# marella/ctransformers

Hardware: NVIDIA H100
Metric: decode tokens/s Llama-2-7B Q4_K_M b=1 (higher is better)
Workload: dtype int8 (q4_K/q6_K weights x q8_K activations, mma.sync u8 x s8 -> exact int32), fp32 combine in the reference's order

## Files before the change

### ctransformers_b200/csrc/attention.cuh

```cuda
#pragma once
#include <cmath>
#include <vector>

#include "device_types.cuh"

namespace ctb {

__device__ __forceinline__ void k4_scale_min(int j, const uint8_t* q, int& sc, int& m) {
  if (j < 4) { sc = q[j] & 63; m = q[j + 4] & 63; }
  else { sc = (q[j + 4] & 0xF) | ((q[j - 4] >> 6) << 4); m = (q[j + 4] >> 4) | ((q[j] >> 6) << 4); }
}

template <bool Q3 = true>
__device__ __forceinline__ float dequant_elem(int type, const uint8_t* row, int e) {
  if (Q3 && type == GT_Q3_K) {
    const uint8_t* blk = row + (size_t)(e >> 8) * 110;
    const int r = e & 255, n = r >> 7, j = (r & 127) >> 5, l = r & 31, is = 8 * n + 2 * j + (l >> 4);
    const int w = is >> 2, b = is & 3;
    const int lo = w & 1 ? blk[100 + b] : blk[96 + b];
    const int sc = ((w < 2 ? lo : lo >> 4) & 0xF) | (((blk[104 + b] >> (2 * w)) & 3) << 4);
    const int q = ((blk[32 + 32 * n + l] >> (2 * j)) & 3) - ((blk[l] >> (4 * n + j)) & 1 ? 0 : 4);
    return __fmul_rn(__fmul_rn(h2f((uint16_t)(blk[108] | (blk[109] << 8))), (float)(sc - 32)), (float)q);
  }
  switch (type) {
    case GT_F32: return ((const float*)row)[e];
    case GT_F16: return h2f(((const uint16_t*)row)[e]);
    case GT_Q4_0: {
      const uint8_t* blk = row + (size_t)(e >> 5) * 18;
      const int r = e & 31;
      const float d = h2f((uint16_t)(blk[0] | (blk[1] << 8)));
      const int byte = blk[2 + (r & 15)];
      const int nib = r < 16 ? (byte & 0xF) : (byte >> 4);
      return __fmul_rn((float)(nib - 8), d);
    }
    case GT_Q5_0: {
      const uint8_t* blk = row + (size_t)(e >> 5) * 22;
      const int r = e & 31;
      const float d = h2f((uint16_t)(blk[0] | (blk[1] << 8)));
      const uint32_t qh = (uint32_t)blk[2] | ((uint32_t)blk[3] << 8) | ((uint32_t)blk[4] << 16) | ((uint32_t)blk[5] << 24);
      const int byte = blk[6 + (r & 15)];
      const int nib = r < 16 ? (byte & 0xF) : (byte >> 4);
      return __fmul_rn((float)((nib | (int)(((qh >> r) & 1u) << 4)) - 16), d);
    }
    case GT_Q4_1: case GT_Q5_1: {
      const bool q5 = type == GT_Q5_1;
      const uint8_t* blk = row + (size_t)(e >> 5) * (q5 ? 24 : 20);
      const int r = e & 31;
      const float d = h2f((uint16_t)(blk[0] | (blk[1] << 8)));
      const float m = h2f((uint16_t)(blk[2] | (blk[3] << 8)));
      const int byte = blk[(q5 ? 8 : 4) + (r & 15)];
      int q = r < 16 ? (byte & 0xF) : (byte >> 4);
      if (q5) q |= ((blk[4 + (r >> 3)] >> (r & 7)) & 1) << 4;
      return __fmaf_rn((float)q, d, m);
    }
    case GT_Q8_0: {
      const uint8_t* blk = row + (size_t)(e >> 5) * 34;
      const float d = h2f((uint16_t)(blk[0] | (blk[1] << 8)));
      return __fmul_rn((float)(int8_t)blk[2 + (e & 31)], d);
    }
    case GT_Q4_K: case GT_Q5_K: {
      const bool q5 = type == GT_Q5_K;
      const uint8_t* blk = row + (size_t)(e >> 8) * (q5 ? 176 : 144);
      const int r = e & 255, j = r >> 6, within = r & 63, sub = 2 * j + (within >> 5), l = within & 31;
      const float d = h2f((uint16_t)(blk[0] | (blk[1] << 8)));
      const float dmin = h2f((uint16_t)(blk[2] | (blk[3] << 8)));
      int sc, m;
      k4_scale_min(sub, blk + 4, sc, m);
      const uint8_t* qs = blk + (q5 ? 48 : 16);
      const int byte = qs[32 * j + l];
      int q = (sub & 1) ? (byte >> 4) : (byte & 0xF);
      if (q5 && (blk[16 + l] & (1 << sub))) q += 16;
      return __fsub_rn(__fmul_rn(__fmul_rn(d, (float)sc), (float)q), __fmul_rn(dmin, (float)m));
    }
    case GT_Q6_K: {
      const uint8_t* blk = row + (size_t)(e >> 8) * 210;
      const uint8_t* ql = blk; const uint8_t* qh = blk + 128; const int8_t* sc = (const int8_t*)(blk + 192);
      const float d = h2f((uint16_t)(blk[208] | (blk[209] << 8)));
      const int r = e & 255, n = r >> 7, rr = r & 127, k = rr >> 5, l = rr & 31, is = l >> 4;
      const int byte = ql[64 * n + ((k & 1) ? 32 : 0) + l];
      const int nib = (k >= 2) ? (byte >> 4) : (byte & 0xF);
      const int hb = (qh[32 * n + l] >> (2 * k)) & 3;
      const int q = (int)(int8_t)(nib | (hb << 4)) - 32;
      return __fmul_rn(__fmul_rn(d, (float)sc[8 * n + is + 2 * k]), (float)q);
    }
  }
  return 0.f;
}

struct EmbedParams { const uint8_t* table; size_t row_bytes; const int* tokens; float* out; int type, K, n_vocab; };

template <bool Q3 = true>
__device__ __forceinline__ void embed_row(const EmbedParams& em, int tok, float* out, int tid, int nt) {
  const uint8_t* row = em.table + (size_t)min(max(tok, 0), em.n_vocab - 1) * em.row_bytes;
  for (int e = tid; e < em.K; e += nt) out[e] = dequant_elem<Q3>(em.type, row, e);
}

static __global__ void k_embed(const EmbedParams em) {
  embed_row(em, em.tokens[blockIdx.x], em.out + (size_t)blockIdx.x * em.K, threadIdx.x, blockDim.x);
}

__host__ __device__ inline int kv_ctx_pad(int n_ctx) { return (n_ctx + 255) & ~255; }
__host__ __device__ inline int k_stride(int hd) { return (hd + 7) & ~7; }
template <bool GEN = true>
__host__ __device__ inline size_t k_row(int kv_head, int pos, int n_ctx, int hd) { return ((size_t)kv_head * n_ctx + pos) * (GEN ? k_stride(hd) : hd); }
__host__ __device__ inline size_t v_chan(int kv_head, int c, int n_ctx, int hd) { return ((size_t)kv_head * hd + c) * kv_ctx_pad(n_ctx); }
template <bool GEN = true>
__host__ __device__ inline int k_perm(int e, int hd) {
  if (!GEN) return (e & 31) * (hd >> 5) + (e >> 5);
  const int np = hd & ~31;
  return e < np ? (e & 31) * (np >> 5) + (e >> 5) : e;
}
__host__ __device__ inline int v_perm(int t) { return (t & ~255) + (t & 31) * 8 + ((t >> 5) & 7); }

inline std::vector<float2> rope_table(int n_pos, int hd, int n_rot, float freq_base, float freq_scale) {
  const int half = hd / 2;
  std::vector<float2> tab((size_t)n_pos * half);
  const float theta_scale = powf(freq_base, -2.0f / n_rot);
  for (int p = 0; p < n_pos; p++) {
    float theta = freq_scale * (float)p;
    for (int i = 0; i < half; i++) {
      tab[(size_t)p * half + i] = make_float2(cosf(theta), sinf(theta));
      theta *= theta_scale;
    }
  }
  return tab;
}

__device__ __forceinline__ void rope_pair(float x0, float x1, float2 cs, int neox, float& o0, float& o1) {
  if (neox) {
    o0 = __fmaf_rn(x0, cs.x, -__fmul_rn(x1, cs.y));
    o1 = __fmaf_rn(x0, cs.y, __fmul_rn(x1, cs.x));
  } else {
    o0 = __fsub_rn(__fmul_rn(x0, cs.x), __fmul_rn(x1, cs.y));
    o1 = __fadd_rn(__fmul_rn(x0, cs.y), __fmul_rn(x1, cs.x));
  }
}

__device__ __forceinline__ void rope_head_pair(const float* x, int i, int hd, int neox, float2 cs, int& i0, int& i1, float& o0, float& o1) {
  i0 = neox ? i : 2 * i;
  i1 = neox ? i + hd / 2 : 2 * i + 1;
  rope_pair(__ldcg(x + i0), __ldcg(x + i1), cs, neox, o0, o1);
}

template <bool GEN = true>
__device__ __forceinline__ void rope_k_pair(const float* x, int i, int hd, int neox, float2 cs, uint16_t* row, uint16_t* row2 = nullptr) {
  int i0, i1;
  float o0, o1;
  rope_head_pair(x, i, hd, neox, cs, i0, i1, o0, o1);
  const uint16_t h0 = f2h(o0), h1 = f2h(o1);
  row[k_perm<GEN>(i0, hd)] = h0; row[k_perm<GEN>(i1, hd)] = h1;
  if (row2) { row2[k_perm<GEN>(i0, hd)] = h0; row2[k_perm<GEN>(i1, hd)] = h1; }
}

struct AttnParams {
  const float* q;
  const float* k;
  const float* v;
  uint16_t* kc;
  uint16_t* vc;
  float* out;
  const uint16_t* exp_tab;
  const float2* rope;
  const int* state;
  float kq_scale;
  int n_head, n_kv, hd, n_ctx, q_stride, kv_stride, neox;
};

constexpr int ATTN_THREADS = 512;
constexpr int ATTN_CH = 32;
__host__ __device__ inline int attn_groups(int hd) { return (hd + ATTN_CH - 1) / ATTN_CH; }

struct AttnScratch { float* sc; uint16_t *p16, *q16, *k16, *v16; size_t bytes; };
template <bool GEN = true>
__host__ __device__ inline AttnScratch attn_scratch(uint8_t* base, int n_ctx, int hd, bool cur) {
  const size_t cp = kv_ctx_pad(n_ctx), ks = GEN ? k_stride(hd) : hd, end_q = cp * 6 + ks * 2;
  AttnScratch s;
  s.sc = (float*)base;
  s.p16 = (uint16_t*)(base + cp * 4);
  s.q16 = s.p16 + cp;
  s.k16 = cur ? s.q16 + ks : nullptr;
  s.v16 = cur ? s.k16 + ks : nullptr;
  s.bytes = cur ? end_q + ks * 2 + (size_t)hd * 2 : end_q;
  return s;
}
__host__ __device__ inline size_t attn_smem_bytes(int n_ctx, int hd) { return attn_scratch(nullptr, n_ctx, hd, true).bytes + (size_t)ATTN_CH * 4; }

__device__ __forceinline__ float attn_reduce_f32x8(float v) {
  v = v + __shfl_xor_sync(0xffffffffu, v, 16);
  v = v + __shfl_xor_sync(0xffffffffu, v, 8);
  v = v + __shfl_xor_sync(0xffffffffu, v, 4);
  v = v + __shfl_xor_sync(0xffffffffu, v, 1);
  v = v + __shfl_xor_sync(0xffffffffu, v, 2);
  return v;
}

template <int BAR, int NT>
__device__ __forceinline__ void attn_bar() {
  if constexpr (NT == 32) __syncwarp();
  else asm volatile("bar.sync %0, %1;" ::"n"(BAR), "n"(NT) : "memory");
}
template <int NT>
__device__ __forceinline__ int attn_tid() { return NT == 32 ? (int)(threadIdx.x & 31) : (int)threadIdx.x; }

struct AttnPos { int pos, T, n_vec, lim; };
__device__ __forceinline__ AttnPos attn_pos(const AttnParams& p, const int* st) {
  AttnPos a;
  a.pos = st[1];
  if (a.pos >= p.n_ctx) { a.T = 0; a.n_vec = 0; a.lim = 0; return a; }
  a.T = a.pos + 1;
  a.n_vec = max(a.T, min(st[3], p.n_ctx)) & ~31;
  a.lim = min(a.T, a.n_vec);
  return a;
}

template <int NT>
__device__ __forceinline__ float2 attn_cs0(const AttnParams& p, int pos) {
  const int i = attn_tid<NT>();
  return i < p.hd / 2 ? p.rope[(size_t)pos * (p.hd / 2) + i] : make_float2(1.f, 0.f);
}

template <int NT, bool GEN>
__device__ __forceinline__ void attn_stage(const AttnParams& p, const AttnScratch& s, int n, int h, int cg, int pos, float2 cs0) {
  const int hd = p.hd, tid = attn_tid<NT>(), group = p.n_head / p.n_kv, kvh = h / group;
  const bool kv_writer = (h % group) == 0;
  const float* qv = p.q + (size_t)n * p.q_stride + (size_t)h * hd;
  const float* kv = p.k + (size_t)n * p.kv_stride + (size_t)kvh * hd;
  const float* vv = p.v + (size_t)n * p.kv_stride + (size_t)kvh * hd;
  uint16_t* kd = (kv_writer && cg == 0) ? p.kc + k_row<GEN>(kvh, pos, p.n_ctx, hd) : nullptr;
  for (int i = tid; i < hd / 2; i += NT) {
    const float2 cs = i == tid ? cs0 : p.rope[(size_t)pos * (hd / 2) + i];
    rope_k_pair<GEN>(qv, i, hd, p.neox, cs, s.q16);
    if (s.k16) rope_k_pair<GEN>(kv, i, hd, p.neox, cs, s.k16, kd);
  }
  if (s.k16) {
    for (int c = tid; c < hd; c += NT) {
      const uint16_t hv = f2h(__ldcg(vv + c));
      s.v16[c] = hv;
      if (kv_writer && c / ATTN_CH == cg) p.vc[v_chan(kvh, c, p.n_ctx, hd) + v_perm(pos)] = hv;
    }
  }
}

template <int PER>
struct KLane { uint32_t w[(PER + 1) / 2]; };
template <int PER>
__device__ __forceinline__ KLane<PER> attn_klane(const uint16_t* row) {
  const uint16_t* p = row + (threadIdx.x & 31) * PER;
  KLane<PER> k;
  if constexpr (PER == 8) {
    const uint4 v = *(const uint4*)p;
    k.w[0] = v.x; k.w[1] = v.y; k.w[2] = v.z; k.w[3] = v.w;
  } else if constexpr (PER == 4) {
    const uint2 v = *(const uint2*)p;
    k.w[0] = v.x; k.w[1] = v.y;
  } else if constexpr (PER % 2 == 0) {
#pragma unroll
    for (int i = 0; i < PER / 2; i++) k.w[i] = ((const uint32_t*)p)[i];
  } else {
#pragma unroll
    for (int i = 0; i < PER / 2; i++) k.w[i] = (uint32_t)p[2 * i] | ((uint32_t)p[2 * i + 1] << 16);
    k.w[PER / 2] = p[PER - 1];
  }
  return k;
}
template <int PER>
__device__ __forceinline__ uint16_t klane_elem(const KLane<PER>& k, int e) { return (uint16_t)((k.w[e >> 1] >> ((e & 1) * 16)) & 0xffff); }
template <int PER>
__device__ __forceinline__ void attn_k8(KLane<PER> (&kk)[8], const uint16_t* rows, int stride, int t0, int n, int skip) {
#pragma unroll
  for (int i = 0; i < 8; i++) {
    const int t = min(t0 + i, n - 1);
    kk[i] = t == skip ? KLane<PER>{} : attn_klane<PER>(rows + (size_t)t * stride);
  }
}

template <int PER, bool TAIL>
__device__ __forceinline__ void attn_scores_per(const uint16_t* rows, int hd, int n, int t_first, int t_step, const uint16_t* q16, float kq_scale, float* sc,
                                                int cur_t, const uint16_t* cur, const KLane<PER> (*pre)[8]) {
  constexpr int NP = PER * 32;
  constexpr int R = PER > 4 ? 4 : 8;
  const int lane = threadIdx.x & 31;
  const int stride = TAIL ? k_stride(hd) : NP, tail = TAIL ? hd - NP : 0;
  const KLane<PER> qq = attn_klane<PER>(q16);
  float q[PER];
#pragma unroll
  for (int e = 0; e < PER; e++) q[e] = h2f(klane_elem(qq, e));
  const float qt = (TAIL && lane < tail) ? h2f(q16[NP + lane]) : 0.f;
  for (int t0 = t_first; t0 < n; t0 += t_step) {
#pragma unroll
    for (int r0 = 0; r0 < 8; r0 += R) {
      KLane<PER> kk[R];
      uint16_t kt[R];
      if (pre && t0 == t_first) {
#pragma unroll
        for (int i = 0; i < R; i++) kk[i] = (*pre)[r0 + i];
      } else {
#pragma unroll
        for (int i = 0; i < R; i++) {
          const int t = min(t0 + r0 + i, n - 1);
          kk[i] = t == cur_t ? KLane<PER>{} : attn_klane<PER>(rows + (size_t)t * stride);
        }
      }
      if constexpr (TAIL) {
#pragma unroll
        for (int i = 0; i < R; i++) {
          const int t = min(t0 + r0 + i, n - 1);
          kt[i] = lane < tail ? (t == cur_t ? cur : rows + (size_t)t * stride)[NP + lane] : (uint16_t)0;
        }
      }
#pragma unroll
      for (int i = 0; i < R; i++)
        if (min(t0 + r0 + i, n - 1) == cur_t) kk[i] = attn_klane<PER>(cur);
#pragma unroll
      for (int i = 0; i < R; i++) {
        float s = 0.f;
#pragma unroll
        for (int e = 0; e < PER; e++) s = __fmaf_rn(h2f(klane_elem(kk[i], e)), q[e], s);
        s = attn_reduce_f32x8(s);
        if constexpr (TAIL) {
          const float term = __fmul_rn(h2f(kt[i]), qt);
          double sumf = (double)s;
          for (int l = 0; l < tail; l++) sumf += (double)__shfl_sync(0xffffffffu, term, l);
          s = (float)sumf;
        }
        if (lane == 0 && t0 + r0 + i < n) sc[t0 + r0 + i] = __fmul_rn(s, kq_scale);
      }
    }
  }
}
#define ATTN_PER_DISPATCH(GEN, hd, F)                             \
  do {                                                            \
    if constexpr (!(GEN)) {                                       \
      if ((hd) == 128) F(4, false);                               \
      else F(2, false);                                           \
    } else {                                                      \
      switch ((hd) >> 5) {                                        \
        case 1: F(1, true); break;                                \
        case 2: F(2, true); break;                                \
        case 3: F(3, true); break;                                \
        case 4: F(4, true); break;                                \
        case 5: F(5, true); break;                                \
        case 6: F(6, true); break;                                \
        case 7: F(7, true); break;                                \
        default: F(8, true); break;                               \
      }                                                           \
    }                                                             \
  } while (0)
template <bool GEN>
__device__ __forceinline__ void attn_scores(int hd, const uint16_t* rows, int n, int t_first, int t_step, const uint16_t* q16, float kq_scale, float* sc,
                                            int cur_t = -1, const uint16_t* cur = nullptr) {
#define ATTN_SCORES_F(PER, TAIL) attn_scores_per<PER, TAIL>(rows, hd, n, t_first, t_step, q16, kq_scale, sc, cur_t, cur, nullptr)
  ATTN_PER_DISPATCH(GEN, hd, ATTN_SCORES_F);
#undef ATTN_SCORES_F
}

template <int NT, int BAR>
__device__ __forceinline__ void attn_softmax(float* sc, uint16_t* p16, int T, const uint16_t* exp_tab, float* red_f, double* red_d) {
  constexpr int NW = NT / 32;
  const int tid = attn_tid<NT>(), warp = tid >> 5, lane = tid & 31;
  float mx = -INFINITY;
  for (int t = tid; t < T; t += NT) mx = fmaxf(mx, sc[t]);
  mx = warp_max(mx);
  if constexpr (NW > 1) {
    if (lane == 0) red_f[warp] = mx;
    attn_bar<BAR, NT>();
    mx = red_f[0];
#pragma unroll
    for (int w = 1; w < NW; w++) mx = fmaxf(mx, red_f[w]);
  }
  double sum = 0.0;
  for (int t = tid; t < T; t += NT) {
    const float val = h2f(__ldg(exp_tab + f2h(__fsub_rn(sc[t], mx))));
    sc[t] = val;
    sum += (double)val;
  }
  sum = warp_sum(sum);
  if constexpr (NW > 1) {
    if (lane == 0) red_d[warp] = sum;
    attn_bar<BAR, NT>();
    sum = 0.0;
#pragma unroll
    for (int w = 0; w < NW; w++) sum += red_d[w];
  }
  const float inv = (float)(1.0 / sum);
  const int t_end = (T + 255) & ~255;
  for (int t = tid; t < t_end; t += NT) p16[v_perm(t)] = t < T ? f2h(__fmul_rn(sc[t], inv)) : (uint16_t)0;
  attn_bar<BAR, NT>();
}

__device__ __forceinline__ float attn_vp(const uint16_t* vrow, const uint16_t* p16, const AttnPos& a, int cur_t, uint16_t vcur, const uint4* pre = nullptr) {
  const int lane = threadIdx.x & 31;
  float s = 0.f;
  for (int ch = 0; ch * 256 < a.lim; ch++) {
    uint4 vv;
    if (pre && ch == 0) vv = pre[0];
    else if (pre && ch == 1) vv = pre[1];
    else vv = *(const uint4*)(vrow + ch * 256 + lane * 8);
    const uint4 pp = *(const uint4*)(p16 + ch * 256 + lane * 8);
    const uint32_t vw[4] = {vv.x, vv.y, vv.z, vv.w}, pw[4] = {pp.x, pp.y, pp.z, pp.w};
#pragma unroll
    for (int i = 0; i < 8; i++) {
      const int t = ch * 256 + 32 * i + lane;
      if (t < a.lim) {
        uint16_t vh = (uint16_t)((vw[i >> 1] >> ((i & 1) * 16)) & 0xffff);
        const uint16_t ph = (uint16_t)((pw[i >> 1] >> ((i & 1) * 16)) & 0xffff);
        if (t == cur_t) vh = vcur;
        s = __fmaf_rn(h2f(vh), h2f(ph), s);
      }
    }
  }
  s = attn_reduce_f32x8(s);
  double sumf = (double)s;
  const int n_left = a.T - a.n_vec;
  if (n_left > 0) {
    const int i = (a.n_vec >> 8) * 256 + lane * 8 + ((a.n_vec & 255) >> 5);
    const uint16_t vh = a.n_vec + lane == cur_t ? vcur : vrow[i];
    const float term = __fmul_rn(h2f(vh), h2f(p16[i]));
    for (int l = 0; l < n_left; l++) sumf += (double)__shfl_sync(0xffffffffu, term, l);
  }
  return (float)sumf;
}

template <int NT, int BAR, bool PDLWAIT, int PER, bool TAIL>
__device__ __forceinline__ void attn_body_per(const AttnParams& p, uint8_t* smem, const int h, const int n, const int cg, const AttnPos& a,
                                              float* red_f, double* red_d) {
  constexpr int NW = NT / 32;
  const int hd = p.hd, kvh = h / (p.n_head / p.n_kv), nch = TAIL ? min(ATTN_CH, hd - cg * ATTN_CH) : ATTN_CH;
  const int warp = threadIdx.x >> 5, lane = threadIdx.x & 31;
  const AttnScratch s = attn_scratch<TAIL>(smem, p.n_ctx, hd, true);
  const uint16_t* krows = p.kc + k_row<TAIL>(kvh, 0, p.n_ctx, hd);
  constexpr int CPW = (ATTN_CH + NW - 1) / NW;
  uint4 vpre[CPW][2];
  constexpr bool KPRE = PER <= 4;
  KLane<PER> kpre[8];
#pragma unroll
  for (int j = 0; j < CPW; j++)
#pragma unroll
    for (int ch = 0; ch < 2; ch++)
      vpre[j][ch] = (ch * 256 < a.lim && warp + j * NW < nch) ? *(const uint4*)(p.vc + v_chan(kvh, cg * ATTN_CH + warp + j * NW, p.n_ctx, hd) + ch * 256 + lane * 8) : make_uint4(0, 0, 0, 0);
  if constexpr (KPRE) attn_k8<PER>(kpre, krows, TAIL ? k_stride(hd) : PER * 32, warp * 8, a.T, a.pos);
  const float2 cs0 = attn_cs0<NT>(p, a.pos);
  if (PDLWAIT) pdl_wait();

  attn_stage<NT, TAIL>(p, s, n, h, cg, a.pos, cs0);
  attn_bar<BAR, NT>();
  attn_scores_per<PER, TAIL>(krows, hd, a.T, warp * 8, NW * 8, s.q16, p.kq_scale, s.sc, a.pos, s.k16, KPRE ? &kpre : nullptr);
  attn_bar<BAR, NT>();
  attn_softmax<NT, BAR>(s.sc, s.p16, a.T, p.exp_tab, red_f, red_d);
#pragma unroll
  for (int j = 0; j < CPW; j++) {
    const int cc = warp + j * NW;
    if (cc >= nch) break;
    const int c = cg * ATTN_CH + cc;
    const float o = attn_vp(p.vc + v_chan(kvh, c, p.n_ctx, hd), s.p16, a, a.pos, s.v16[c], vpre[j]);
    if (lane == 0) p.out[(size_t)n * p.n_head * hd + (size_t)h * hd + c] = o;
  }
}
template <int NT>
__device__ __forceinline__ void attn_body_red(float*& red_f, double*& red_d) {
  __shared__ float rf[NT / 32];
  __shared__ double rd[NT / 32];
  red_f = rf;
  red_d = rd;
}
template <int NT, int BAR, bool PDLWAIT, bool GEN>
__device__ __forceinline__ void attn_body(const AttnParams& p, uint8_t* smem, const int h, const int n, const int cg, const int* st) {
  float* red_f;
  double* red_d;
  attn_body_red<NT>(red_f, red_d);
  const AttnPos a = attn_pos(p, st);
  if (a.T == 0) return;
#define ATTN_BODY_F(PER, TAIL) attn_body_per<NT, BAR, PDLWAIT, PER, TAIL>(p, smem, h, n, cg, a, red_f, red_d)
  ATTN_PER_DISPATCH(GEN, p.hd, ATTN_BODY_F);
#undef ATTN_BODY_F
}

template <bool GEN>
static __global__ void __launch_bounds__(ATTN_THREADS) k_attn(const AttnParams p) {
  extern __shared__ __align__(16) uint8_t smem[];
  pdl_trigger();
  attn_body<ATTN_THREADS, 0, true, GEN>(p, smem, blockIdx.x, blockIdx.y, blockIdx.z, p.state);
}
inline void (*attn_kernel(int hd))(const AttnParams) { return attn_fast_hd(hd) ? k_attn<false> : k_attn<true>; }

template <int NT, int BAR, bool CG>
__device__ __forceinline__ void block_argmax(const float* logits, int n, float* bv , int* bi , float& best, int& idx) {
  best = -INFINITY;
  idx = 0x7fffffff;
#pragma unroll(CG ? 4 : 1)
  for (int i = threadIdx.x; i < n; i += NT) {
    const float v = CG ? __ldcg(logits + i) : logits[i];
    if (v > best) { best = v; idx = i; }
  }
#pragma unroll
  for (int o = 16; o > 0; o >>= 1) {
    const float ov = __shfl_xor_sync(0xffffffffu, best, o);
    const int oi = __shfl_xor_sync(0xffffffffu, idx, o);
    if (ov > best || (ov == best && oi < idx)) { best = ov; idx = oi; }
  }
  if ((threadIdx.x & 31) == 0) { bv[threadIdx.x >> 5] = best; bi[threadIdx.x >> 5] = idx; }
  bar_sync<BAR, NT>();
  if (threadIdx.x == 0) {
    for (int w = 1; w < NT / 32; w++)
      if (bv[w] > best || (bv[w] == best && bi[w] < idx)) { best = bv[w]; idx = bi[w]; }
    const float x0 = CG ? __ldcg(logits) : logits[0];
    if (idx == 0x7fffffff || x0 != x0) { best = x0; idx = 0; }
  }
}

__device__ __forceinline__ void advance_state(int* state, int* out_tokens, int pick) {
  out_tokens[state[2]] = pick;
  state[0] = pick;
  state[1] += 1;
  state[2] += 1;
  state[3] = state[1] + 1;
}

constexpr int ARGMAX_THREADS = 1024;
static __global__ void k_argmax(const float* logits, int n, int* out) {
  __shared__ float bv[ARGMAX_THREADS / 32];
  __shared__ int bi[ARGMAX_THREADS / 32];
  __shared__ int ties;
  float best;
  int idx;
  block_argmax<ARGMAX_THREADS, 0, false>(logits, n, bv, bi, best, idx);
  if (threadIdx.x == 0) {
    out[0] = idx;
    bv[0] = best;
    ties = 0;
  }
  __syncthreads();
  const float top = bv[0];
  int mine = 0;
  for (int i = threadIdx.x; i < n; i += blockDim.x) mine += logits[i] == top ? 1 : 0;
  if (mine) atomicAdd(&ties, mine);
  __syncthreads();
  if (threadIdx.x == 0) out[1] = ties;
}

}
```

### ctransformers_b200/csrc/stream.cuh

```cuda
#pragma once
#include "matvec.cuh"

namespace ctb {

#ifndef CTB_ST_WARPS
#define CTB_ST_WARPS 10
#endif
constexpr int ST_W = CTB_ST_WARPS;
constexpr int ST_NT = ST_W * 32;
constexpr int ST_THREADS = ST_NT + 32;
constexpr int ST_SLOT = 9216;
#ifndef CTB_ST_DEPTH
#define CTB_ST_DEPTH 2
#endif
constexpr int ST_MAX_DEPTH = CTB_ST_DEPTH;
constexpr int ST_MAX_SLOTS = ST_W * ST_MAX_DEPTH;
constexpr int ST_MAXT = 16;
constexpr int ST_ROWS = 16;
constexpr int ST_BAR = 1;
constexpr int ST_STATE = 6;

#ifndef CTB_CHUNK_Q3
#define CTB_CHUNK_Q3 5
#endif
// ... 371 lines not shown
      const int i = rr * 2 + c;
      r.p[i] = (float)scale_fold8(D[0][i], D[1][i], D[2][i], D[3][i], D[4][i], D[5][i], D[6][i], D[7][i], S0, S1);
    }
    r.dd[rr] = __fmul_rn(yd, h2f(rr ? d1 : d0));
  }
}

template <int TYPE, bool XC>
__device__ __forceinline__ void run_item(const uint8_t* slot, uint64_t* empty_bar, int nblk, int b0, int kc, bool last, const StAct& a, int lane,
                                         volatile float* mail, volatile int* flag, const MVSeg& sg, const MVParams& p, int row0) {
  constexpr int KB = StTraits<TYPE>::KB, BB = StTraits<TYPE>::BB, NM = StTraits<TYPE>::NM;
  Terms tr[KB];
  if (nblk == KB) {
#pragma unroll
    for (int i = 0; i < KB; i++) block_terms<TYPE>(slot + i * BB, b0 + i, a, lane, tr[i]);
  } else {
#pragma unroll
    for (int i = 0; i < KB; i++) {
      if (i < nblk) block_terms<TYPE>(slot + i * BB, b0 + i, a, lane, tr[i]);
      else { Terms z{}; tr[i] = z; }
    }
  }
  __syncwarp();
  if (lane == 0) mbar_arrive(empty_bar);

  float acc[4] = {0.f, 0.f, 0.f, 0.f}, accm[2] = {0.f, 0.f};
  if (kc > 0) {
    if (lane == 0) bounded_wait([&] { return *flag >= kc; }, W_FOLD_FLAG, kc);
    __syncwarp();
    __threadfence_block();
#pragma unroll
    for (int i = 0; i < 4; i++) acc[i] = mail[i * 32 + lane];
#pragma unroll
    for (int i = 0; i < NM; i++) accm[i] = mail[(4 + i) * 32 + lane];
  }
#pragma unroll
  for (int i = 0; i < KB; i++) {
    if (i < nblk) {
#pragma unroll
      for (int q = 0; q < 4; q++) acc[q] = __fmaf_rn(tr[i].dd[q >> 1], tr[i].p[q], acc[q]);
#pragma unroll
      for (int q = 0; q < NM; q++) accm[q] = __fmaf_rn(tr[i].ddm[q], tr[i].pm[q], accm[q]);
    }
  }
  if (!last) {
    __syncwarp();
#pragma unroll
    for (int i = 0; i < 4; i++) mail[i * 32 + lane] = acc[i];
#pragma unroll
    for (int i = 0; i < NM; i++) mail[(4 + i) * 32 + lane] = accm[i];
    __threadfence_block();
    __syncwarp();
    if (lane == 0) *flag = kc + 1;
    return;
  }
  const int t = lane & 3, g = lane >> 2;
  float out[2];
#pragma unroll
  for (int rr = 0; rr < 2; rr++) {
    float u0 = acc[rr * 2], u1 = acc[rr * 2 + 1];
    u0 = __fadd_rn(u0, __shfl_xor_sync(0xffffffffu, u0, 2));
    u1 = __fadd_rn(u1, __shfl_xor_sync(0xffffffffu, u1, 2));
    u0 = __fadd_rn(u0, __shfl_xor_sync(0xffffffffu, u0, 1));
    u1 = __fadd_rn(u1, __shfl_xor_sync(0xffffffffu, u1, 1));
    float v = __fadd_rn(u0, u1);
    if (TYPE == GT_Q4_K) {
      float m = accm[rr];
      m = __fadd_rn(m, __shfl_xor_sync(0xffffffffu, m, 2));
      m = __fadd_rn(m, __shfl_xor_sync(0xffffffffu, m, 1));
      v = __fadd_rn(v, m);
    } else if (TYPE == GT_Q5_K) {
      v = __fadd_rn(v, __shfl_sync(0xffffffffu, accm[0], (lane & ~3) + rr));
    }
    out[rr] = v;
  }
  if (t < 2) {
    const int row = row0 + g + 8 * t;
    if (row < sg.w.M) {
      if (XC && a.xc) {
        const float v = epilogue(sg.epi, t ? out[1] : out[0], sg.res + row, sg.res2 + row, p);
        const XchgParams& xc = *a.xc;
        const size_t at = ((size_t)(a.epoch & 1u) * xc.world + xc.rank) * xc.n + row;
        for (int r = 0; r < xc.world; r++)
          asm volatile("st.volatile.global.v2.u32 [%0], {%1, %2};" ::"l"(xc.ll[r] + at), "r"(__float_as_uint(v)), "r"(a.epoch) : "memory");
      } else {
        store_epilogue(sg, p, row, t ? out[1] : out[0]);
      }
    }
  }
}

struct TileSpace {
  int tiles[MV_MAX_SEG], cost[MV_MAX_SEG], nseg, ntiles;
  long total;
  template <bool Q3 = true>
  __host__ __device__ __forceinline__ void init(const MVParams& p) {
    nseg = p.nseg; ntiles = 0; total = 0;
#pragma unroll
    for (int s = 0; s < MV_MAX_SEG; s++) {
      tiles[s] = s < p.nseg ? (p.seg[s].w.M + ST_ROWS - 1) / ST_ROWS : 0;
      cost[s] = s < p.nseg ? st_tile_cost<Q3>(p.seg[s].w.type) : 1;
      ntiles += tiles[s]; total += (long)tiles[s] * cost[s];
    }
  }
  __host__ __device__ __forceinline__ int locate(int& tile) const {
    static_assert(MV_MAX_SEG == 3, "locate() is written out for three segments");
    if (tile < tiles[0]) return 0;
    tile -= tiles[0];
    if (tile < tiles[1]) return 1;
    tile -= tiles[1];
    return 2;
  }
  __host__ __device__ __forceinline__ int boundary(int c, int G) const {
    if (c >= G) return ntiles;
    long target = total * c / G;
    int base = 0;
#pragma unroll
    for (int s = 0; s < MV_MAX_SEG; s++) {
      const long span = (long)tiles[s] * cost[s];
      if (target < span || s == MV_MAX_SEG - 1) return base + (int)min((long)tiles[s], (target + cost[s] / 2) / cost[s]);
      target -= span; base += tiles[s];
    }
    return ntiles;
  }
};

enum : int { PH_MATVEC = 0, PH_ATTN = 1, PH_EMBED = 2, PH_PICK = 3,
              PH_XCHG = 4 };
constexpr int XC_MAX_WORLD = 8;
struct XchgParams {
  int world, rank, index, n;
  int role;
  uint2* ll[XC_MAX_WORLD];
};
struct PickParams { const float* logits; int* state; int* out_tokens; int n; };
struct alignas(16) Phase {
  int kind;
  int q6;
  MVParams mv;
  AttnParams at;
  EmbedParams em;
  PickParams pk;
  XchgParams xc;
};

struct StepArgs {
  const Phase* prog;
  int n_phases;
  int n_slots;
  unsigned* sync;
  const int* bounds;
  unsigned long long* trace;
};

__device__ __forceinline__ unsigned ld_relaxed_u32(const unsigned* p) {
  unsigned v;
  asm volatile("ld.relaxed.gpu.global.u32 %0, [%1];" : "=r"(v) : "l"(p) : "memory");
  return v;
}
__device__ __forceinline__ unsigned ld_acquire_u32(const unsigned* p) {
  unsigned v;
  asm volatile("ld.acquire.gpu.global.u32 %0, [%1];" : "=r"(v) : "l"(p) : "memory");
  return v;
}

struct TileInfo { int seg, til, nch, type; };
template <bool Q3>
__device__ __forceinline__ TileInfo tile_info(const TileSpace& ts, const MVParams& p, int tile, int nb, bool valid) {
  TileInfo ti;
  ti.seg = 0; ti.til = 0; ti.nch = 0; ti.type = GT_Q4_K;
  if (valid) {
    int tl = tile;
    ti.seg = ts.locate(tl);
    ti.til = tl;
    ti.type = ti.seg == 0 ? p.seg[0].w.type : (ti.seg == 1 ? p.seg[1].w.type : p.seg[2].w.type);
    ti.nch = st_chunks<Q3>(ti.type, nb);
  }
  return ti;
}

struct StItem { const uint8_t* src; uint32_t bytes; };
template <bool Q3>
__device__ __forceinline__ StItem st_item(const MVParams& p, int seg, int type, int til, int kc, int nb) {
  const int kb = st_chunk_blocks<Q3>(type), bb = st_block_bytes<Q3>(type);
  const int nblk = min(kb, nb - kc * kb);
  const uint8_t* base = seg == 0 ? p.seg[0].w.st : (seg == 1 ? p.seg[1].w.st : p.seg[2].w.st);
  return {base + ((size_t)til * nb + (size_t)kc * kb) * bb, (uint32_t)(nblk * bb)};
}

struct AttnRingV { int nchv, cv, n_v; };
__host__ __device__ inline AttnRingV attn_ring_v(int T) {
  AttnRingV v;
  v.nchv = (T + 255) >> 8;
  v.cv = max(1, min(8, ST_SLOT / (v.nchv * 512)));
  v.n_v = (ATTN_CH + v.cv - 1) / v.cv;
  return v;
}
struct AttnRing : AttnPos, AttnRingV { int n_k, rpi; };
template <bool GEN>
__device__ __forceinline__ AttnRing attn_ring_geom(const AttnParams& p) {
  AttnRing g;
  static_cast<AttnPos&>(g) = attn_pos(p, p.state);
  g.rpi = ST_SLOT / ((GEN ? k_stride(p.hd) : p.hd) * 2);
  if (g.T == 0) { g.n_k = 0; g.n_v = 0; g.cv = 1; g.nchv = 0; return g; }
  static_cast<AttnRingV&>(g) = attn_ring_v(g.T);
  g.n_k = (g.pos + g.rpi - 1) / g.rpi;
  return g;
}
__device__ __forceinline__ int attn_group_ch(int hd, int cg) { return min(ATTN_CH, hd - cg * ATTN_CH); }
template <bool GEN>
__device__ __forceinline__ int attn_ring_nv(const AttnRing& g, int hd, int cg) { return GEN && g.n_v > 0 ? (attn_group_ch(hd, cg) + g.cv - 1) / g.cv : g.n_v; }

template <bool GEN>
__device__ __forceinline__ void st_attn_produce(const AttnParams& p, uint8_t* ring, uint64_t* full_bar, uint64_t* empty_bar, uint32_t S, uint32_t& seq) {
  const int lane = threadIdx.x & 31;
  const AttnRing g = attn_ring_geom<GEN>(p);
  const int n_cg = GEN ? attn_groups(p.hd) : p.hd / ATTN_CH, n_tasks = p.n_head * n_cg, group = p.n_head / p.n_kv, row_bytes = (GEN ? k_stride(p.hd) : p.hd) * 2;
  for (int task = blockIdx.x; task < n_tasks; task += gridDim.x) {
    const int h = task / n_cg, cg = task % n_cg, kvh = h / group;
    const int step = min(32, ST_W * (int)S);
    for (int i0 = 0; i0 < g.n_k; i0 += step) {
      const int i = i0 + lane;
      if (lane < step && i < g.n_k) {
        const uint32_t n = seq + (uint32_t)i;
        const RingPos rp = st_ring(n, S);
        const int rows = min(g.rpi, g.pos - i * g.rpi);
        mbar_wait(&empty_bar[rp.slot], rp.parity ^ 1u, W_FREE_K_SLOT, (int)n);
        mbar_expect_tx(&full_bar[rp.slot], (uint32_t)(rows * row_bytes));
        bulk_g2s(ring + (size_t)rp.slot * ST_SLOT, p.kc + k_row<GEN>(kvh, i * g.rpi, p.n_ctx, p.hd), (uint32_t)(rows * row_bytes), &full_bar[rp.slot]);
      }
      __syncwarp();
    }
    seq += (uint32_t)g.n_k;
    const int n_v = attn_ring_nv<GEN>(g, p.hd, cg), ch_g = GEN ? attn_group_ch(p.hd, cg) : ATTN_CH;
    for (int iv = lane; iv < n_v; iv += 32) {
      const uint32_t n = seq + (uint32_t)iv;
      const RingPos rp = st_ring(n, S);
      const int nch = min(g.cv, ch_g - iv * g.cv);
      const uint32_t bytes = (uint32_t)(g.nchv * 512);
      mbar_wait(&empty_bar[rp.slot], rp.parity ^ 1u, W_FREE_V_SLOT, (int)n);
      mbar_expect_tx(&full_bar[rp.slot], bytes * nch);
      for (int q = 0; q < nch; q++)
        bulk_g2s(ring + (size_t)rp.slot * ST_SLOT + (size_t)q * bytes, p.vc + v_chan(kvh, cg * ATTN_CH + iv * g.cv + q, p.n_ctx, p.hd), bytes,
                 &full_bar[rp.slot]);
    }
    __syncwarp();
    seq += (uint32_t)n_v;
  }
}

template <bool GEN>
__device__ __forceinline__ void st_attn_task(const AttnParams& p, uint8_t* smem, const uint8_t* ring, uint64_t* full_bar, uint64_t* empty_bar, uint32_t S, uint32_t seq0,
                                             const AttnRing& g, int h, int cg, float* red_f, double* red_d) {
  const int warp = threadIdx.x >> 5, lane = threadIdx.x & 31, nch = GEN ? attn_group_ch(p.hd, cg) : ATTN_CH;
  const AttnScratch s = attn_scratch<GEN>(smem, p.n_ctx, p.hd, true);
  attn_stage<ST_NT, GEN>(p, s, 0, h, cg, g.pos, attn_cs0<ST_NT>(p, g.pos));
  bar_sync<ST_BAR, ST_NT>();
  for (int i = (int)(((uint32_t)warp + ST_W - seq0 % ST_W) % ST_W); i < g.n_k; i += ST_W) {
    const uint32_t n = seq0 + (uint32_t)i;
    const RingPos rp = st_ring(n, S);
    const int r0 = i * g.rpi;
    mbar_wait(&full_bar[rp.slot], rp.parity, W_K_ITEM, (int)n);
    attn_scores<GEN>(p.hd, (const uint16_t*)(ring + (size_t)rp.slot * ST_SLOT), min(g.rpi, g.pos - r0), 0, 8, s.q16, p.kq_scale, s.sc + r0);
    __syncwarp();
    if (lane == 0) mbar_arrive(&empty_bar[rp.slot]);
  }
  if (warp == (int)((seq0 + (uint32_t)g.n_k) % ST_W)) attn_scores<GEN>(p.hd, s.k16, 1, 0, 8, s.q16, p.kq_scale, s.sc + g.pos);
  bar_sync<ST_BAR, ST_NT>();
  attn_softmax<ST_NT, ST_BAR>(s.sc, s.p16, g.T, p.exp_tab, red_f, red_d);
  for (int cc = warp; cc < nch; cc += ST_W) {
    const int c = cg * ATTN_CH + cc;
    const uint32_t n = seq0 + (uint32_t)(g.n_k + cc / g.cv);
    const RingPos rp = st_ring(n, S);
    mbar_wait(&full_bar[rp.slot], rp.parity, W_V_ITEM, (int)n);
    const uint16_t* vrow = (const uint16_t*)(ring + (size_t)rp.slot * ST_SLOT + (size_t)(cc % g.cv) * g.nchv * 512);
    const float o = attn_vp(vrow, s.p16, g, g.pos, s.v16[c]);
    if (lane == 0) p.out[(size_t)h * p.hd + c] = o;
  }
  bar_sync<ST_BAR, ST_NT>();
  if ((int)threadIdx.x < attn_ring_nv<GEN>(g, p.hd, cg)) {
    const uint32_t n = seq0 + (uint32_t)(g.n_k + threadIdx.x);
    mbar_arrive(&empty_bar[st_ring(n, S).slot]);
  }
}

template <bool GEN>
__device__ __forceinline__ void st_attn_phase(const Phase& ph, uint8_t* act_smem, uint8_t* ring, uint64_t* full_bar, uint64_t* empty_bar, int n_slots,
                                              uint32_t& seq, float* pick_v, double* red) {
  const int n_cg = GEN ? attn_groups(ph.at.hd) : ph.at.hd / ATTN_CH, n_tasks = ph.at.n_head * n_cg, G = (int)gridDim.x;
  if (ph.q6) {
    const AttnRing ag = attn_ring_geom<GEN>(ph.at);
    for (int task = blockIdx.x; task < n_tasks; task += G) {
      if (task != (int)blockIdx.x) bar_sync<ST_BAR, ST_NT>();
      if (ag.T > 0) st_attn_task<GEN>(ph.at, act_smem, ring, full_bar, empty_bar, (uint32_t)(n_slots / ST_W), seq, ag, task / n_cg, task % n_cg, pick_v, red);
      seq += (uint32_t)(ag.n_k + attn_ring_nv<GEN>(ag, ph.at.hd, task % n_cg));
    }
  } else {
    for (int task = blockIdx.x; task < n_tasks; task += G) {
      if (task != (int)blockIdx.x) bar_sync<ST_BAR, ST_NT>();
      attn_body<ST_NT, ST_BAR, false, GEN>(ph.at, act_smem, task / n_cg, 0, task % n_cg, ph.at.state);
    }
  }
}
template <bool Q3>
static __device__ __noinline__ uint32_t st_attn_phase_gen(const Phase& ph, uint8_t* act_smem, uint8_t* ring, uint64_t* full_bar, uint64_t* empty_bar, int n_slots,
                                                   uint32_t seq, float* pick_v, double* red) {
  st_attn_phase<true>(ph, act_smem, ring, full_bar, empty_bar, n_slots, seq, pick_v, red);
  return seq;
}

template <bool XC, bool GEN, bool Q3>
__device__ __forceinline__ void st_producer(const StepArgs& args, uint8_t* ring, uint64_t* full_bar, uint64_t* empty_bar) {
  const int lane = threadIdx.x & 31;
  const uint32_t S = (uint32_t)(args.n_slots / ST_W);
  const uint64_t weight_pol = l2_policy_evict_first();
  uint32_t seq = 0;
  for (int ip = 0; ip < args.n_phases; ip++) {
    const Phase* ph = args.prog + ip;
    if (ph->kind == PH_ATTN) {
      if (ph->q6) {
        if (GEN) st_attn_produce<true>(ph->at, ring, full_bar, empty_bar, S, seq);
        else st_attn_produce<false>(ph->at, ring, full_bar, empty_bar, S, seq);
      }
      continue;
    }
    if (ph->kind != PH_MATVEC) continue;
    const MVParams& p = ph->mv;
    TileSpace ts;
    ts.init<Q3>(p);
    const int* bnd = args.bounds + (size_t)ip * (gridDim.x + 1) + blockIdx.x;
    const int T0 = __ldg(bnd), T1 = __ldg(bnd + 1);
    const int nb = p.K >> 8;
    for (int w0 = T0; w0 < T1; w0 += ST_MAXT) {
      const int ntw = min(ST_MAXT, T1 - w0);
      const TileInfo ti = tile_info<Q3>(ts, p, w0 + lane, nb, lane < ntw);
      for (int kc = 0;; kc++) {
        const unsigned mask = __ballot_sync(0xffffffffu, kc < ti.nch);
        if (!mask) break;
        const int rank = __popc(mask & ((1u << lane) - 1u)), cnt = __popc(mask);
        for (int base = 0; base < cnt; base += ST_W * (int)S) {
          if (((mask >> lane) & 1u) && rank >= base && rank < base + ST_W * (int)S) {
            const uint32_t n = seq + (uint32_t)rank;
            const RingPos rp = st_ring(n, S);
            const StItem it = st_item<Q3>(p, ti.seg, ti.type, ti.til, kc, nb);
            mbar_wait(&empty_bar[rp.slot], rp.parity ^ 1u, W_FREE_WEIGHT_SLOT, (int)n);
            mbar_expect_tx(&full_bar[rp.slot], it.bytes);
            bulk_g2s_hint(ring + (size_t)rp.slot * ST_SLOT, it.src, it.bytes, &full_bar[rp.slot], weight_pol);
          }
          __syncwarp();
        }
        __syncwarp();
        seq += (uint32_t)__popc(mask);
      }
    }
  }
}

template <bool XC, bool Q3>
__device__ __forceinline__ void st_matvec_phase(const Phase& ph, const NormPre& np, uint8_t* ring, uint8_t* act_smem, double* red, uint64_t* full_bar, uint64_t* empty_bar,
                                                float (*mailbox)[ST_STATE * 32], int* flags, uint32_t S, uint32_t& seq, const int* tb, unsigned long long* tr,
                                                unsigned xc_base) {
  const MVParams& p = ph.mv;
  const int warp = threadIdx.x >> 5, lane = threadIdx.x & 31;
  const unsigned epoch = XC ? xc_base + (unsigned)ph.xc.index + 1u : 0u;
  stage_activation<ST_NT, ST_BAR, XC>(p, np, ACT_Q8_K, act_smem, red, blockIdx.x == 0, epoch);
  StAct a = st_act_extras<ST_NT, ST_BAR>(act_smem, p.K, ph.q6 != 0);
  a.xc = XC && ph.xc.role == 2 ? &ph.xc : nullptr;
  a.epoch = epoch;
  if (tr && threadIdx.x == 0) tr[1] = globaltimer_ns();
  bool first_item = tr != nullptr && threadIdx.x == 0;
  TileSpace ts;
  ts.init<Q3>(p);
  const int nb = p.K >> 8;
  const int T0 = tb[0], T1 = tb[1];
#pragma unroll 1
  for (int w0 = T0; w0 < T1; w0 += ST_MAXT) {
    if (w0 != T0) {
      bar_sync<ST_BAR, ST_NT>();
      if (threadIdx.x < ST_MAXT) flags[threadIdx.x] = 0;
      bar_sync<ST_BAR, ST_NT>();
    }
    const int ntw = min(ST_MAXT, T1 - w0);
    const TileInfo ti = tile_info<Q3>(ts, p, w0 + lane, nb, lane < ntw);
#pragma unroll 1
    for (int kc = 0;; kc++) {
      const unsigned mask = __ballot_sync(0xffffffffu, kc < ti.nch);
      if (!mask) break;
      const int cnt = __popc(mask);
#pragma unroll 1
      for (int r = (int)(((uint32_t)warp + ST_W - seq % ST_W) % ST_W); r < cnt; r += ST_W) {
        unsigned mr = mask;
        for (int q = 0; q < r; q++) mr &= mr - 1;
        const int j = __ffs(mr) - 1;
        const int seg = __shfl_sync(0xffffffffu, ti.seg, j), til = __shfl_sync(0xffffffffu, ti.til, j), type = __shfl_sync(0xffffffffu, ti.type, j);
        const int nch = __shfl_sync(0xffffffffu, ti.nch, j);
        const uint32_t n = seq + (uint32_t)r;
        const RingPos rp = st_ring(n, S);
        const int kb = st_chunk_blocks<Q3>(type);
        const int b0 = kc * kb, nblk = min(kb, nb - b0);
        const MVSeg& sg = p.seg[seg];
        const uint8_t* sp = ring + (size_t)rp.slot * ST_SLOT;
        mbar_wait(&full_bar[rp.slot], rp.parity, W_WEIGHT_ITEM, (int)n);
        if (first_item) { tr[2] = globaltimer_ns(); first_item = false; }
        volatile float* mail = mailbox[j];
        volatile int* flag = flags + j;
        const bool last = kc == nch - 1;
        if (type == GT_Q4_K) run_item<GT_Q4_K, XC>(sp, &empty_bar[rp.slot], nblk, b0, kc, last, a, lane, mail, flag, sg, p, til * ST_ROWS);
        else if (type == GT_Q6_K) run_item<GT_Q6_K, XC>(sp, &empty_bar[rp.slot], nblk, b0, kc, last, a, lane, mail, flag, sg, p, til * ST_ROWS);
        else if (Q3 && type == GT_Q3_K) run_item<GT_Q3_K, XC>(sp, &empty_bar[rp.slot], nblk, b0, kc, last, a, lane, mail, flag, sg, p, til * ST_ROWS);
        else run_item<GT_Q5_K, XC>(sp, &empty_bar[rp.slot], nblk, b0, kc, last, a, lane, mail, flag, sg, p, til * ST_ROWS);
      }
      seq += (uint32_t)cnt;
    }
  }
}

__device__ __forceinline__ void st_pick_phase(const PickParams& pk, float* bv, int* bi) {
  float best;
  int idx;
  block_argmax<ST_NT, ST_BAR, true>(pk.logits, pk.n, bv, bi, best, idx);
  if (threadIdx.x == 0) {
    pk.state[4] = idx;
    advance_state(pk.state, pk.out_tokens, idx);
  }
}

__device__ __forceinline__ void grid_rearm(unsigned* sync, bool set_xc = false, unsigned xc = 0) {
  if (threadIdx.x == 0) {
    __threadfence();
    if (atomicAdd(sync + 1, 1u) == gridDim.x - 1) {
      sync[0] = 0u;
      sync[1] = 0u;
      if (set_xc) sync[2] = xc;
      __threadfence();
    }
  }
}

template <bool XC, bool GEN, bool Q3>
static __global__ void __launch_bounds__(ST_THREADS, 1) k_step(const __grid_constant__ StepArgs args) {
  extern __shared__ __align__(16) uint8_t smem[];
  __shared__ __align__(8) uint64_t full_bar[ST_MAX_SLOTS];
  __shared__ __align__(8) uint64_t empty_bar[ST_MAX_SLOTS];
  __shared__ double red[3 * ST_W];
  __shared__ __align__(16) float mailbox[ST_MAXT][ST_STATE * 32];
  __shared__ int flags[ST_MAXT];
  __shared__ float pick_v[ST_W];
  __shared__ int pick_i[ST_W];
  __shared__ __align__(16) Phase ph_s[2];
  __shared__ int tb_s[2][2];
  const int warp = threadIdx.x >> 5;
  uint8_t* ring = smem;
  uint8_t* act_smem = smem + (size_t)args.n_slots * ST_SLOT;
  ring_init(full_bar, empty_bar, args.n_slots, 1);
  pdl_trigger();
  pdl_wait();
  if (warp == ST_W) {
    st_producer<XC, GEN, Q3>(args, ring, full_bar, empty_bar);
    return;
  }
  const unsigned G = gridDim.x;
  uint32_t seq = 0;
  const unsigned xc_base = XC ? ld_relaxed_u32(args.sync + 2) : 0u;
  unsigned xc_done = 0;
  auto fetch_phase = [&](int ip) {
    if (ip >= args.n_phases) return;
    const uint4* src = (const uint4*)(args.prog + ip);
    const uint32_t dst = st_smem(&ph_s[ip & 1]);
    const int i = (int)threadIdx.x - 32;
    if (i >= 0 && i < (int)(sizeof(Phase) / 16)) asm volatile("cp.async.ca.shared.global [%0], [%1], 16;" ::"r"(dst + i * 16), "l"(src + i) : "memory");
    if (i >= 64 && i < 66)
      asm volatile("cp.async.ca.shared.global [%0], [%1], 4;" ::"r"(st_smem(&tb_s[ip & 1][i - 64])), "l"(args.bounds + (size_t)ip * (gridDim.x + 1) + blockIdx.x + (i - 64)) : "memory");
    asm volatile("cp.async.commit_group;" ::: "memory");
  };
  fetch_phase(0);
#pragma unroll 1
  for (int ip = 0; ip < args.n_phases; ip++) {
    bar_sync<ST_BAR, ST_NT>();
    unsigned long long* const tr = args.trace ? args.trace + ((size_t)ip * G + blockIdx.x) * 8 : nullptr;
    if (tr && threadIdx.x == 0) tr[4] = globaltimer_ns();
    if (threadIdx.x == 0 && ip > 0) {
      const unsigned target = (unsigned)ip * G;
      asm volatile("red.release.gpu.global.add.u32 [%0], 1;" ::"l"(args.sync) : "memory");
      if (tr) tr[5] = globaltimer_ns();
      bounded_wait([&] { return ld_relaxed_u32(args.sync) >= target; }, W_GRID_BARRIER, ip);
      if (tr) { tr[6] = globaltimer_ns(); tr[7] = tr[6]; }
    } else {
      asm volatile("cp.async.wait_all;" ::: "memory");
      if (threadIdx.x >= 32 && threadIdx.x < 32 + ST_MAXT) flags[threadIdx.x - 32] = 0;
    }
    bar_sync<ST_BAR, ST_NT>();
    const Phase& ph = ph_s[ip & 1];
    fetch_phase(ip + 1);
    NormPre np;
    if (ph.kind == PH_MATVEC) preload_norm(np, ph.mv);
    if (tr && threadIdx.x == 0) tr[0] = globaltimer_ns();
    if (XC && ph.kind == PH_MATVEC && ph.xc.role == 1) xc_done++;
    if (ph.kind == PH_MATVEC) {
      st_matvec_phase<XC, Q3>(ph, np, ring, act_smem, red, full_bar, empty_bar, mailbox, flags, (uint32_t)(args.n_slots / ST_W), seq, &tb_s[ip & 1][0], tr, xc_base);
    } else if (ph.kind == PH_ATTN) {
      if (GEN) seq = st_attn_phase_gen<Q3>(ph, act_smem, ring, full_bar, empty_bar, args.n_slots, seq, pick_v, red);
      else st_attn_phase<false>(ph, act_smem, ring, full_bar, empty_bar, args.n_slots, seq, pick_v, red);
    } else if (ph.kind == PH_EMBED) {
      if (blockIdx.x == 0) embed_row<Q3>(ph.em, ph.em.tokens[0], ph.em.out, threadIdx.x, ST_NT);
    } else if (ph.kind == PH_PICK) {
      if (blockIdx.x == 0) st_pick_phase(ph.pk, pick_v, pick_i);
    }
    if (tr) {
      bar_sync<ST_BAR, ST_NT>();
      if (threadIdx.x == 0) tr[3] = globaltimer_ns();
    }
  }
  bar_sync<ST_BAR, ST_NT>();
  grid_rearm(args.sync, XC, xc_base + xc_done);
}

struct StepLaunch { int grid; int n_slots; size_t smem; bool gen = false, q3 = false;  };

inline StepLaunch step_launch_shape(const Phase* phases, int n, int n_sm, size_t max_dyn_smem, size_t extra_act = 0) {
  size_t act = extra_act;
  for (int i = 0; i < n; i++) {
    if (phases[i].kind == PH_MATVEC) act = std::max(act, st_act_bytes(phases[i].mv.K, phases[i].q6 != 0));
    if (phases[i].kind == PH_ATTN) act = std::max(act, attn_smem_bytes(phases[i].at.n_ctx, phases[i].at.hd));
  }
  bool gen = false, q3 = false;
  for (int i = 0; i < n; i++) {
    gen |= phases[i].kind == PH_ATTN && !attn_fast_hd(phases[i].at.hd);
    if (phases[i].kind == PH_MATVEC)
      for (int s = 0; s < phases[i].mv.nseg; s++) q3 |= phases[i].mv.seg[s].w.type == GT_Q3_K;
    q3 |= phases[i].kind == PH_EMBED && phases[i].em.type == GT_Q3_K;
  }
  act = (act + 127) & ~(size_t)127;
  StepLaunch L;
  L.grid = n_sm;
  L.gen = gen;
  L.q3 = q3;
  if (act + (size_t)ST_W * ST_SLOT > max_dyn_smem) { L.n_slots = 0; L.smem = 0; return L; }
  L.n_slots = ST_W * (int)std::min<size_t>(ST_MAX_DEPTH, (max_dyn_smem - act) / ((size_t)ST_W * ST_SLOT));
  L.smem = (size_t)L.n_slots * ST_SLOT + act;
  return L;
}

inline std::vector<int> step_bounds(const Phase* phs, int n, int grid) {
  std::vector<int> b((size_t)n * (grid + 1), 0);
  for (int i = 0; i < n; i++) {
    if (phs[i].kind != PH_MATVEC) continue;
    TileSpace ts;
    ts.init(phs[i].mv);
    for (int c = 0; c <= grid; c++) b[(size_t)i * (grid + 1) + c] = ts.boundary(c, grid);
  }
  return b;
}

inline bool st_attn_ring_ok(int n_ctx, int n_slots) { return attn_ring_v(n_ctx).n_v <= n_slots; }

inline bool step_supports(const MVParams& p) {
  if (p.K % 256) return false;
  for (int s = 0; s < p.nseg; s++)
    if (!type_is_kquant(p.seg[s].w.type) || !p.seg[s].w.st) return false;
  return p.nseg >= 1;
}
inline Phase matvec_phase(const MVParams& p) {
  Phase ph{};
  ph.kind = PH_MATVEC;
  ph.mv = p;
  ph.mv.act = ACT_Q8_K;
  for (int s = 0; s < p.nseg; s++) ph.q6 |= p.seg[s].w.type == GT_Q6_K || p.seg[s].w.type == GT_Q3_K;
  return ph;
}

static inline cudaError_t st_set_debug_words(int* dev_ptr) { return cudaMemcpyToSymbol(g_st_dbg, &dev_ptr, sizeof(int*)); }
static inline cudaError_t step_set_smem_limit(size_t bytes) {
  void (*const kernels[])(StepArgs) = {k_step<false, false, false>, k_step<false, true, false>, k_step<true, false, false>,
                                        k_step<false, false, true>, k_step<false, true, true>, k_step<true, false, true>};
  for (auto k : kernels) {
    const cudaError_t e = cudaFuncSetAttribute(k, cudaFuncAttributeMaxDynamicSharedMemorySize, (int)bytes);
    if (e != cudaSuccess) return e;
  }
  return cudaSuccess;
}

static inline cudaError_t launch_step(const StepLaunch& L, cudaStream_t st, const Phase* d_prog, const int* d_bounds, int n_phases, unsigned* d_sync, bool pdl = false,
                                      unsigned long long* trace = nullptr, bool xchg = false) {
  StepArgs a;
  a.prog = d_prog; a.bounds = d_bounds; a.n_phases = n_phases; a.n_slots = L.n_slots; a.sync = d_sync; a.trace = trace;
  auto kernel = L.q3 ? (xchg ? k_step<true, false, true> : (L.gen ? k_step<false, true, true> : k_step<false, false, true>))
                     : (xchg ? k_step<true, false, false> : (L.gen ? k_step<false, true, false> : k_step<false, false, false>));
  return launch_kernel(kernel, dim3(L.grid), dim3(ST_THREADS), L.smem, st, pdl, a);
}

}
```

Before: 359.4.

## Batch QK score warp reductions across 8 rows and outline attention phase

For the non-tail, eight-row case of the QK score loop, the eight per-row warp reductions are replaced by one transpose-style butterfly reduction. Each shuffle then carries a useful partial for a different row, which cuts the shuffle count from 40 to 10 per group, and lanes with (lane&3)==0 write one score each. Separately, the attention phase call is now always a noinline function, including the non-GEN path, with the aim of reducing register pressure and code size in the persistent kernel. The trade-off is extra select instructions and an extra call overhead on the previously inlined path; the floating-point summation order also changes.

```diff
diff --git a/ctransformers_b200/csrc/attention.cuh b/ctransformers_b200/csrc/attention.cuh
--- a/ctransformers_b200/csrc/attention.cuh
+++ b/ctransformers_b200/csrc/attention.cuh
@@ -194,6 +194,24 @@
   return v;
 }
 
+__device__ __forceinline__ float attn_reduce8_f32x8(float (&x)[8]) {
+  const int lane = threadIdx.x & 31;
+#pragma unroll
+  for (int lv = 0; lv < 3; lv++) {
+    const int m = 16 >> lv, h = 4 >> lv;
+    const bool up = (lane & m) != 0;
+#pragma unroll
+    for (int i = 0; i < h; i++) {
+      const float keep = up ? x[i + h] : x[i], send = up ? x[i] : x[i + h];
+      x[i] = keep + __shfl_xor_sync(0xffffffffu, send, m);
+    }
+  }
+  float v = x[0];
+  v = v + __shfl_xor_sync(0xffffffffu, v, 1);
+  v = v + __shfl_xor_sync(0xffffffffu, v, 2);
+  return v;
+}
+
 template <int BAR, int NT>
 __device__ __forceinline__ void attn_bar() {
   if constexpr (NT == 32) __syncwarp();
@@ -311,19 +329,32 @@
 #pragma unroll
       for (int i = 0; i < R; i++)
         if (min(t0 + r0 + i, n - 1) == cur_t) kk[i] = attn_klane<PER>(cur);
-#pragma unroll
-      for (int i = 0; i < R; i++) {
-        float s = 0.f;
-#pragma unroll
-        for (int e = 0; e < PER; e++) s = __fmaf_rn(h2f(klane_elem(kk[i], e)), q[e], s);
-        s = attn_reduce_f32x8(s);
-        if constexpr (TAIL) {
-          const float term = __fmul_rn(h2f(kt[i]), qt);
-          double sumf = (double)s;
-          for (int l = 0; l < tail; l++) sumf += (double)__shfl_sync(0xffffffffu, term, l);
-          s = (float)sumf;
+      if constexpr (!TAIL && R == 8) {
+        float x[8];
+#pragma unroll
+        for (int i = 0; i < 8; i++) {
+          x[i] = 0.f;
+#pragma unroll
+          for (int e = 0; e < PER; e++) x[i] = __fmaf_rn(h2f(klane_elem(kk[i], e)), q[e], x[i]);
         }
-        if (lane == 0 && t0 + r0 + i < n) sc[t0 + r0 + i] = __fmul_rn(s, kq_scale);
+        const float s = attn_reduce8_f32x8(x);
+        const int t = t0 + r0 + ((lane >> 2) & 7);
+        if ((lane & 3) == 0 && t < n) sc[t] = __fmul_rn(s, kq_scale);
+      } else {
+#pragma unroll
+        for (int i = 0; i < R; i++) {
+          float s = 0.f;
+#pragma unroll
+          for (int e = 0; e < PER; e++) s = __fmaf_rn(h2f(klane_elem(kk[i], e)), q[e], s);
+          s = attn_reduce_f32x8(s);
+          if constexpr (TAIL) {
+            const float term = __fmul_rn(h2f(kt[i]), qt);
+            double sumf = (double)s;
+            for (int l = 0; l < tail; l++) sumf += (double)__shfl_sync(0xffffffffu, term, l);
+            s = (float)sumf;
+          }
+          if (lane == 0 && t0 + r0 + i < n) sc[t0 + r0 + i] = __fmul_rn(s, kq_scale);
+        }
       }
     }
   }
diff --git a/ctransformers_b200/csrc/stream.cuh b/ctransformers_b200/csrc/stream.cuh
--- a/ctransformers_b200/csrc/stream.cuh
+++ b/ctransformers_b200/csrc/stream.cuh
@@ -697,10 +697,10 @@
     }
   }
 }
-template <bool Q3>
-static __device__ __noinline__ uint32_t st_attn_phase_gen(const Phase& ph, uint8_t* act_smem, uint8_t* ring, uint64_t* full_bar, uint64_t* empty_bar, int n_slots,
-                                                   uint32_t seq, float* pick_v, double* red) {
-  st_attn_phase<true>(ph, act_smem, ring, full_bar, empty_bar, n_slots, seq, pick_v, red);
+template <bool XC, bool GEN, bool Q3>
+static __device__ __noinline__ uint32_t st_attn_phase_call(const Phase& ph, uint8_t* act_smem, uint8_t* ring, uint64_t* full_bar, uint64_t* empty_bar, int n_slots,
+                                                           uint32_t seq, float* pick_v, double* red) {
+  st_attn_phase<GEN>(ph, act_smem, ring, full_bar, empty_bar, n_slots, seq, pick_v, red);
   return seq;
 }
 
@@ -894,8 +894,7 @@
     if (ph.kind == PH_MATVEC) {
       st_matvec_phase<XC, Q3>(ph, np, ring, act_smem, red, full_bar, empty_bar, mailbox, flags, (uint32_t)(args.n_slots / ST_W), seq, &tb_s[ip & 1][0], tr, xc_base);
     } else if (ph.kind == PH_ATTN) {
-      if (GEN) seq = st_attn_phase_gen<Q3>(ph, act_smem, ring, full_bar, empty_bar, args.n_slots, seq, pick_v, red);
-      else st_attn_phase<false>(ph, act_smem, ring, full_bar, empty_bar, args.n_slots, seq, pick_v, red);
+      seq = st_attn_phase_call<XC, GEN, Q3>(ph, act_smem, ring, full_bar, empty_bar, args.n_slots, seq, pick_v, red);
     } else if (ph.kind == PH_EMBED) {
       if (blockIdx.x == 0) embed_row<Q3>(ph.em, ph.em.tokens[0], ph.em.out, threadIdx.x, ST_NT);
     } else if (ph.kind == PH_PICK) {
```

After: 362.3 (median of 6 runs). About the same (+0.8%).
